# pdh930105/ARCQuant

Measured on AMD Instinct MI355X. Metric: ARC-NVFP4 GEMM TFLOP/s (M=4096, N=KQ=4096, KE=64), higher is better.
Workload: dtype f16

## Files before the change

arcquant_amd/agemm.py:

```python
from __future__ import annotations

import functools

import torch

from . import _lib
from ._lib import VARIANT_G16, VARIANT_G32, OUT_BF16, OUT_F32, ArcqError

_raw_stream = getattr(torch._C, "_cuda_getCurrentRawStream", None)


def _stream(t: torch.Tensor) -> int:
    if _raw_stream is not None:
        return _raw_stream(t.get_device())
    return torch.cuda.current_stream(t.device).cuda_stream


class _on:
    __slots__ = ("ctx",)

    def __init__(self, device):
        idx = device.index
        self.ctx = None if idx is None or idx == torch.cuda.current_device() else torch.cuda.device(device)

# ... 1 lines not shown
        if self.ctx is not None:
            self.ctx.__enter__()

    def __exit__(self, *exc):
        if self.ctx is not None:
            return self.ctx.__exit__(*exc)
        return False



def _need(t: torch.Tensor, dtype, name: str, ndim=None):
    if getattr(t, "dtype", None) is not dtype:
        raise RuntimeError(f"agemm: {name} must be a {dtype} tensor, got {getattr(t, 'dtype', type(t))}")
    if ndim is not None and t.dim() != ndim:
        raise RuntimeError(f"agemm: {name} must be {ndim}-D, got shape {tuple(t.shape)}")
    if not t.is_contiguous():
        raise RuntimeError(f"agemm: {name} must be contiguous")


def _opt(t, dtype, name, shape):
    if t is None:
        return None
    _need(t, dtype, name, len(shape))
    if t.shape != shape:
        raise RuntimeError(f"agemm: {name} must have shape {shape}")
    return t.data_ptr()


def _slots(t, who):
    if t is None:
        return None, 0
    _need(t, torch.int32, "absmax_slots", 1)
    if t.numel() == 0:
        raise RuntimeError(f"agemm.{who}: absmax_slots must not be empty")
    return t.data_ptr(), t.numel()


def _alpha(scale, scale_host):
    if isinstance(scale, torch.Tensor) and scale.is_cuda and scale.dtype == torch.float32 and scale.numel() == 1:
        return float(scale_host), scale, scale.data_ptr()
    return float(scale_host) * float(scale), None, None


def _alpha_as_f32(scale, scale_host):
    if isinstance(scale, torch.Tensor) and scale.is_cuda:
        scale = scale.reshape(-1)[:1].to(torch.float32)
        return float(scale_host), scale, scale.data_ptr()
    return float(scale_host) * float(scale), None, None


_OUT_CODES = {torch.bfloat16: OUT_BF16, torch.float32: OUT_F32}


def _out(out, M, N, out_dtype, like, who):
    code = _OUT_CODES.get(out_dtype)
    if code is None:
        raise RuntimeError(f"agemm.{who}: out_dtype must be bfloat16 or float32")
    if out is None:
        return torch.empty((M, N), dtype=out_dtype, device=like.device), code
    _need(out, out_dtype, "out", 2)
    if out.shape != (M, N):
        raise RuntimeError(f"agemm.{who}: out has the wrong shape, expected ({M}, {N})")
    return out, code


def _same_device(who: str, A: torch.Tensor, *ts):
    idx = A.get_device()
    if idx < 0:
        raise RuntimeError(f"agemm.{who}: the operands must live on the GPU (there is no CPU path)")
    for t in ts:
        if t is not None and t.get_device() != idx:
            raise RuntimeError(f"agemm.{who}: every operand must live on the GPU of the first one ({A.device}), got {t.device}")


def _debug_set_tile_overlap_tail(mode: int) -> None:
    fn = _lib.lib().arcq_debug_set_tile_overlap_tail
    fn.restype, fn.argtypes = None, [_lib._i32]
    fn(int(mode))
    rw_route.cache_clear()


def _debug_set_tile_pair_loads(on: int) -> None:
    fn = _lib.lib().arcq_debug_set_tile_pair_loads
    fn.restype, fn.argtypes = None, [_lib._i32]
    fn(int(on))


@functools.lru_cache(maxsize=None)
def variant_for_kq(KQ: int) -> int:
    return int(_lib.lib().arcq_variant_for_kq(int(KQ)))


@functools.lru_cache(maxsize=None)
def sf_buffer_bytes(rows: int, K: int) -> int:
    return int(_lib.lib().arcq_sf_alloc_bytes(int(rows), int(K)))


@functools.lru_cache(maxsize=None)
def _sf_used(rows: int, K: int) -> int:
    return int(_lib.lib().arcq_sf_used_bytes(int(rows), int(K)))


@functools.lru_cache(maxsize=None)
def _repacked_bytes(N: int, K: int):
    L = _lib.lib()
    return int(L.arcq_repacked_w_bytes(N, K)), int(L.arcq_repacked_sf_bytes(N, K))


def _need_repacked(RW, RSF, SFA, M, N, K, who, n_mult=1):
    _need(RW, torch.uint8, "RW", 1)
    _need(RSF, torch.uint8, "RSF", 1)
    if K % 64 or N % n_mult or (RW.numel(), RSF.numel()) != _repacked_bytes(N, K):
        raise RuntimeError(f"Value error in {who}: RW / RSF do not belong to a [{N}, {K}] weight" + (f", or N % {n_mult} != 0" if n_mult > 1 else ""))
    if SFA is not None and SFA.numel() < _sf_used(M, K):
        raise RuntimeError(f"Value error in {who}: SFA smaller than the swizzled layout of A")


def _quantize(fn_name: str, X: torch.Tensor, reorder_index: torch.Tensor, KE: int, variant):
    _need(X, torch.bfloat16, "X" if fn_name.endswith("_x") else "W", 2)
    _need(reorder_index, torch.int16, "reorder_index", 1)
    rows, KQ = X.shape
    KE = int(KE)
    if reorder_index.numel() != KQ:
        raise RuntimeError(f"agemm: reorder_index has {reorder_index.numel()} entries, expected {KQ}")
    K = KQ + KE
    if variant is None:
        variant = variant_for_kq(KQ)
    if KQ % 64 or KE % 64 or KE < 0 or KE > KQ:
        raise RuntimeError(f"Value error in {fn_name}: KQ={KQ}, KE={KE} is not valid")
    _same_device(fn_name, X, reorder_index)
    Q = torch.empty((rows, K // 2), dtype=torch.uint8, device=X.device)
    SF = torch.empty((sf_buffer_bytes(rows, K),), dtype=torch.uint8, device=X.device)
    L = _lib.lib()
    fn = L.arcq_quantize_x if fn_name.endswith("_x") else L.arcq_quantize_w
    with _on(X.device):
        st = fn(X.data_ptr(), reorder_index.data_ptr(), Q.data_ptr(), SF.data_ptr(), rows, KQ, KE, int(variant), _stream(X))
    _lib.check(st, fn_name)
    return Q, SF


def reorder_quantize_x(X: torch.Tensor, reorder_index: torch.Tensor, KE: int, variant=None):
    return _quantize("reorder_quantize_x", X, reorder_index, KE, variant)


def reorder_quantize_w(W: torch.Tensor, reorder_index: torch.Tensor, KE: int, variant=None):
    return _quantize("reorder_quantize_w", W, reorder_index, KE, variant)


def rmsnorm_quantize_x(X: torch.Tensor, W: torch.Tensor, eps: float, reorder_index: torch.Tensor, KE: int, variant=None):
    _need(X, torch.bfloat16, "X", 2)
    _need(W, torch.bfloat16, "W", 1)
    _need(reorder_index, torch.int16, "reorder_index", 1)
    M, KQ = X.shape
    KE = int(KE)
    K = KQ + KE
    if W.numel() != KQ or reorder_index.numel() != KQ:
        raise RuntimeError("agemm: rmsnorm weight / reorder_index length must equal X.shape[1]")
    if variant is None:
        variant = variant_for_kq(KQ)
    if KQ % 64 or KE % 64 or KE < 0 or KE > KQ or not (2048 <= KQ <= 8192):
        raise RuntimeError(f"Value error in run_rmsnorm_x_bf16_nvfp4: K value is not valid: {KQ}")
    _same_device("rmsnorm_quantize_x", X, W, reorder_index)
    QX = torch.empty((M, K // 2), dtype=torch.uint8, device=X.device)
    SFX = torch.empty((sf_buffer_bytes(M, K),), dtype=torch.uint8, device=X.device)
    with _on(X.device):
        st = _lib.lib().arcq_rmsnorm_quantize_x(X.data_ptr(), W.data_ptr(), float(eps), reorder_index.data_ptr(), QX.data_ptr(),
# ... 427 lines not shown
```

arcquant_amd/csrc/arcq_internal.hpp:

```cpp
#pragma once
#include <hip/hip_runtime.h>
#include <stdint.h>
#include <stdlib.h>

#include "../../include/arcq.h"

namespace arcq {

int fail(int code, const char* fmt, ...) __attribute__((format(printf, 2, 3)));

inline int env_int(const char* name, int dflt) {
  const char* e = getenv(name);
  return e ? atoi(e) : dflt;
}

constexpr int kMaxDevices = 64;
struct LdsOptIn {
  int granted[kMaxDevices];
};
int ensure_dynamic_lds(const void* kernel, LdsOptIn& cache, int bytes, const char* who);

struct LdsBytes {
  int launch, optin;
  LdsBytes(int bytes) : launch(bytes), optin(bytes) {}
// ... 42 lines not shown
int mx_quantize_w(const void* W, const int16_t* idx, uint8_t* QW, uint8_t* SFW, int64_t N, int64_t KQ, int64_t KE, hipStream_t stream);
int gemm_mx(const uint8_t* A, const uint8_t* B, const uint8_t* SFA, const uint8_t* SFB, void* D, int64_t M, int64_t N, int64_t Kp,
            float alpha_host, const float* alpha_dev, const void* bias, const void* residual, int out_dtype, hipStream_t stream);
int mx_rmsnorm_quantize_x(const void* X, const void* Wn, float eps, const int16_t* idx, uint8_t* QX, uint8_t* SFX, int64_t M, int64_t KQ,
                          int64_t KE, hipStream_t stream);
int mx_silu_mul_quantize_x(const void* GU, const int16_t* idx, uint8_t* QX, uint8_t* SFX, int64_t M, int64_t KQ, int64_t KE, int layout,
                           hipStream_t stream);
int gemm_mx_silu_mul(const uint8_t* A, const uint8_t* B, const uint8_t* SFA, const uint8_t* SFB, void* ACT, int64_t M, int64_t N, int64_t Kp,
                     float alpha_host, const float* alpha_dev, const void* bias, hipStream_t stream);
int gemm_mx_silu_mul_quantize(const uint8_t* A, const uint8_t* B, const uint8_t* SFA, const uint8_t* SFB, uint8_t* QACT, uint8_t* SFACT, int64_t M,
                              int64_t N, int64_t Kp, float alpha_host, const float* alpha_dev, const void* bias, int64_t KE, hipStream_t stream);

struct GemmArgs {
  const uint8_t* A;
  const uint8_t* B;
  const uint8_t* SFA;
  const uint8_t* SFB;
  void* D;
  int M, N, K;
  float alpha_host;
  const float* alpha_dev;
  const uint16_t* bias;
  const uint16_t* residual;
  int out_dtype;
  void* workspace;
  int64_t workspace_bytes;
  int epilogue = 0;
  unsigned int* absmax_slots = nullptr;
  int b_layout = 0;
};
template <typename Params>
void copy_gemm_fields(Params& p, const GemmArgs& a) {
  p.A = a.A; p.SFA = a.SFA; p.D = a.D;
  p.alpha_dev = a.alpha_dev; p.bias = a.bias; p.residual = a.residual;
  p.M = a.M; p.N = a.N; p.K = a.K; p.alpha_host = a.alpha_host; p.out_dtype = a.out_dtype;
}
enum : int { kEpiPlain = 0, kEpiSiluMul = 1 };
enum : int { kBRef = 0, kBRepacked = 1 };
int64_t gemm_silu_slots(int64_t M, int64_t N, int64_t K);
int64_t gemm_repacked_w_bytes(int64_t N, int64_t K);
int64_t gemm_repacked_sf_bytes(int64_t N, int64_t K);
int gemm_repacked_supported(int64_t M, int64_t N, int64_t K);
int gemm_repacked(const GemmArgs& a, const uint8_t* RW, const uint8_t* RSF, hipStream_t stream);
int gemm_repacked_mid_supported(int64_t M, int64_t N, int64_t K);
int gemm_repacked_mid(const GemmArgs& a, const uint8_t* RW, const uint8_t* RSF, hipStream_t stream);
int gemm_repacked_stream(const GemmArgs& a, const uint8_t* RW, const uint8_t* RSF, hipStream_t stream);
struct FusedArgs {
  int kind;
  int silu_act;
  const uint16_t* X;
  const uint16_t* Wn;
  float eps;
  const int16_t* idx;
  const uint32_t* in_slots;
  int n_in_slots;
  float* scale_out;
  const uint8_t* RW;
  const uint8_t* RSF;
  void* D;
  uint32_t* out_slots;
  const int16_t* act_scatter;
  int M, N, KQ, KE, variant;
  float alpha_host;
  const float* alpha_dev;
  const uint16_t* bias;
  const uint16_t* residual;
  int out_dtype;
};
int gemm_fused_supported(int kind, int64_t M, int64_t N, int64_t KQ, int64_t KE);
int gemm_fused(const FusedArgs& f, hipStream_t stream);
int64_t gemm_skinny_workspace_bytes(int64_t M, int64_t N, int64_t K);
int64_t gemm_tile_workspace_bytes(int64_t M, int64_t N, int64_t K);
int64_t gemm_tile_silu_slots(int64_t M, int64_t N, int64_t K);
int64_t gemm_decode_silu_slots(int64_t M, int64_t N, int64_t K);
int gemm_splitk_finish(const GemmArgs& a, int splitk, hipStream_t stream);
int gemm_skinny(const GemmArgs& a, hipStream_t stream);
int64_t gemm_decode_workspace_bytes(int64_t M, int64_t N, int64_t K);
int gemm_decode(const GemmArgs& a, hipStream_t stream);
int gemm_tile(const GemmArgs& a, hipStream_t stream);
int gemm_tile_repacked(const GemmArgs& a, hipStream_t stream);
int tile_overlap_tail_mode();
inline bool tile_overlap_tail_forced(int64_t M, int64_t N) { return tile_overlap_tail_mode() == 2 && M % 256 == 0 && N % 256 == 0; }
int tile_pair_loads_mode();
int gemm_regtile_cfg(int64_t M, int64_t N, int64_t K, int epilogue);
int gemm_regtile(const GemmArgs& a, int cfg, hipStream_t stream);
int gemm_regtile_fits(int64_t M, int64_t N, int64_t K, int b_layout);

struct KvWriteArgs {
  void* kv_data;
  void* kv_param;
  const int32_t *kv_indptr, *kv_indices, *last_page_offset;
  const void *k, *v, *k_param, *v_param;
  const int32_t* seqlen_indptr;
  int64_t ntok, B, L, layer, N, P;
  int format, dtype;
  bool quantize;
};
int kv_write(const KvWriteArgs& a, hipStream_t stream);
struct KvDecodeArgs {
  void* o;
  const void *q, *kv_data, *kv_param;
  const int32_t *kv_indptr, *kv_indices, *last_page_offset;
  int64_t B, Nq, L, layer, N, P, nnz;
  int format, dtype;
  void* workspace;
};
int kv_decode_splits(int64_t B, int64_t Nq, int64_t N, int64_t nnz, int64_t P);
int kv_decode(const KvDecodeArgs& a, hipStream_t stream);
struct KvStepArgs {
  const void *k, *v;
  int64_t q_stride, kv_stride;
  void* state;
};
int64_t kv_decode_chunks(int64_t Nq, int64_t N);
int kv_decode_step(const KvDecodeArgs& a, const KvStepArgs& st, hipStream_t stream);

struct KvPrefillArgs {
  void* o;
  const void* q;
  const int32_t* qo_indptr;
  const void *kv_data, *kv_param;
  const int32_t *kv_indptr, *kv_indices, *last_page_offset;
  int64_t ntok, B, Nq, L, layer, N, P;
  int dtype;
};
int kv_prefill(const KvPrefillArgs& a, hipStream_t stream);

struct KvRopeArgs {
  KvWriteArgs w;
  void* q_out;
  const void* q;
  const void *cos, *sin;
  int64_t q_stride, kv_stride, Nq;
  const char* who;
};
int kv_rope_write(const KvRopeArgs& a, hipStream_t stream);
struct RopeQkArgs {
  void *q, *k;
  const int32_t* positions;
  const void *cos, *sin;
  int64_t q_stride, k_stride, ntok, n_pos, Nq, N;
  int dtype;
};
int kv_rope_qk(const RopeQkArgs& a, hipStream_t stream);

}
```

arcquant_amd/csrc/gemm_tile_body.inc:

```
  constexpr int kThreads = WAVES_M * WAVES_N * 64;
  constexpr int WM = BM / WAVES_M, WN = BN / WAVES_N;
  constexpr int kT = kMfma32 ? 32 : 16;
  constexpr int TM = WM / kT, TN = WN / kT;
  using acc_t = typename std::conditional<kMfma32, f32x16, f32x4>::type;
  constexpr int A_UNITS = (BM * 2 + kThreads - 1) / kThreads, B_UNITS = (BN * 2 + kThreads - 1) / kThreads;
  constexpr bool A_PARTIAL = (BM * 2) % kThreads != 0, B_PARTIAL = (BN * 2) % kThreads != 0;
  static_assert(!A_PARTIAL || A_UNITS == 1, "a partial A pass is a single pass");
  static_assert(!B_PARTIAL || B_UNITS == 1, "a partial B pass is a single pass");
  constexpr int A_TILE = BM * kRowBytes, B_TILE = BN * kRowBytes;

  extern __shared__ __attribute__((aligned(16))) unsigned char smem[];
  unsigned char* const lds_a0 = smem;
  unsigned char* const lds_b0 = smem + A_TILE;
  unsigned char* const lds_a1 = smem + A_TILE + B_TILE;
  unsigned char* const lds_b1 = smem + 2 * A_TILE + B_TILE;

  const int ntiles = p.tiles_m * p.tiles_n;
  int bid = blockIdx.x, split = 0;
  if (p.splits > 1) {
    split = bid / ntiles;
    bid -= split * ntiles;
  }
  {
    const int q8 = ntiles >> 3, r8 = ntiles & 7, x = bid & 7, j = bid >> 3;
// ... 51 lines not shown
  int b_slot[B_UNITS][4];
#pragma unroll
  for (int u = 0; u < B_UNITS; ++u) {
    const int unit = tid + u * kThreads, r = B_PARTIAL ? min(unit >> 1, BN - 1) : unit >> 1, h = unit & 1;
    const int row = n0 + r, rc = row < p.N ? row : p.N - 1;
    if constexpr (kBLayout == kBRepacked) {
      const uint32_t rb = (uint32_t)((rc >> 4) - (n0 >> 4));
      b_q[u] = rb * (uint32_t)rw_tiles * 1024u + h * 256 + (rc & 15) * 16;
      b_sf[u] = rb * (uint32_t)rw_tiles * 128u + h * 64 + (rc & 15) * 4;
    } else {
      b_q[u] = (uint32_t)(rc - n0) * (uint32_t)half_k + h * 16;
      b_sf[u] = (uint32_t)(sf_atom_offset(rc, 0, atoms_k) - sf_atom_offset(n0, 0, atoms_k)) + h * 2;
    }
    b_live[u] = row < p.N ? kSfLive : 0u;
#pragma unroll
    for (int j = 0; j < 4; ++j) b_slot[u][j] = kMfma32 ? lds_slot32(r, h * 4 + j) : lds_slot(r, h * 4 + j);
  }
  const int fa_base = kMfma32 ? lds_slot32(wr * WM + (lane & 31), lane >> 5) : lds_slot(wr * WM + (lane & 15), lane >> 4);
  const int fb_base = kMfma32 ? lds_slot32(wc * WN + (lane & 31), lane >> 5) : lds_slot(wc * WN + (lane & 15), lane >> 4);
  acc_t acc[TM][TN];
  if constexpr (!kOverlapTail) {
#pragma unroll
    for (int i = 0; i < TM; ++i)
#pragma unroll
      for (int j = 0; j < TN; ++j)
#pragma unroll
        for (int r = 0; r < (kMfma32 ? 16 : 4); ++r) acc[i][j][r] = 0.f;
  }

  Staged sa[A_UNITS], sb[B_UNITS];
  auto load_step = [&](int atom) {
    atom = __builtin_amdgcn_readfirstlane(atom);
    const StageStep sa_step = stage_step(atom), sb_step = kBLayout == kBRepacked ? stage_step_rw(atom) : sa_step;
#pragma unroll
    for (int u = 0; u < A_UNITS; ++u) sa[u] = stage_load(a_src, a_q[u], a_sf[u], sa_step);
#pragma unroll
    for (int u = 0; u < B_UNITS; ++u) sb[u] = stage_load(b_src, b_q[u], b_sf[u], sb_step);
  };
#ifdef ARCQ_TILE_BODY_PAIR_LOADS
  Staged sa2[A_UNITS], sb2[B_UNITS];
  auto load_pair = [&](int atom0, int atom1, Staged (&a0)[A_UNITS], Staged (&b0)[B_UNITS], Staged (&a1)[A_UNITS], Staged (&b1)[B_UNITS], auto parts) {
    constexpr int kParts = decltype(parts)::value;
    atom0 = __builtin_amdgcn_readfirstlane(atom0);
    atom1 = __builtin_amdgcn_readfirstlane(atom1);
    const StageStep a_s0 = stage_step(atom0), a_s1 = stage_step(atom1);
    const StageStep b_s0 = kBLayout == kBRepacked ? stage_step_rw(atom0) : a_s0, b_s1 = kBLayout == kBRepacked ? stage_step_rw(atom1) : a_s1;
    __builtin_amdgcn_sched_barrier(0);
    if constexpr ((kParts & 1) != 0) {
#pragma unroll
      for (int u = 0; u < A_UNITS; ++u) {
        a0[u].q = stage_load_q(a_src, a_q[u], a_s0);
        __builtin_amdgcn_sched_barrier(0);
        a1[u].q = stage_load_q(a_src, a_q[u], a_s1);
        __builtin_amdgcn_sched_barrier(0);
      }
    }
    if constexpr ((kParts & 2) != 0) {
#pragma unroll
      for (int u = 0; u < B_UNITS; ++u) {
        b0[u].q = stage_load_q(b_src, b_q[u], b_s0);
        __builtin_amdgcn_sched_barrier(0);
        b1[u].q = stage_load_q(b_src, b_q[u], b_s1);
        __builtin_amdgcn_sched_barrier(0);
      }
    }
    if constexpr ((kParts & 4) != 0) {
#pragma unroll
      for (int u = 0; u < A_UNITS; ++u) {
        a0[u].sf = stage_load_sf(a_src, a_sf[u], a_s0);
        a1[u].sf = stage_load_sf(a_src, a_sf[u], a_s1);
      }
#pragma unroll
      for (int u = 0; u < B_UNITS; ++u) {
        b0[u].sf = stage_load_sf(b_src, b_sf[u], b_s0);
        b1[u].sf = stage_load_sf(b_src, b_sf[u], b_s1);
      }
    }
  };
  using kPairA = std::integral_constant<int, 1>;
  using kPairB = std::integral_constant<int, 2>;
  using kPairSf = std::integral_constant<int, 4>;
  using kPairAll = std::integral_constant<int, 7>;
#endif
  auto store_step = [&](unsigned char* la, unsigned char* lb) {
#pragma unroll
    for (int u = 0; u < A_UNITS; ++u)
      if (!A_PARTIAL || tid < BM * 2) stage_store(la, a_slot[u], sa[u], a_live[u]);
#pragma unroll
    for (int u = 0; u < B_UNITS; ++u)
      if (!B_PARTIAL || tid < BN * 2) stage_store(lb, b_slot[u], sb[u], b_live[u]);
  };
  auto mma_step = [&](const unsigned char* la, const unsigned char* lb) {
    if constexpr (kMfma32) {
#pragma unroll
      for (int ks = 0; ks < 4; ++ks) {
        Frag8 fa[TM], fb[TN];
#pragma unroll
        for (int i = 0; i < TM; ++i) fa[i].u = *reinterpret_cast<const uint4*>(la + (fa_base ^ (ks * 32)) + i * 32 * kRowBytes);
#pragma unroll
        for (int j = 0; j < TN; ++j) fb[j].u = *reinterpret_cast<const uint4*>(lb + (fb_base ^ (ks * 32)) + j * 32 * kRowBytes);
#pragma unroll
        for (int i = 0; i < TM; ++i)
#pragma unroll
          for (int j = 0; j < TN; ++j) acc[i][j] = __builtin_amdgcn_mfma_f32_32x32x16_f16(fb[j].v, fa[i].v, acc[i][j], 0, 0, 0);
      }
    } else {
#pragma unroll
      for (int ks = 0; ks < 2; ++ks) {
        Frag8 fa[TM], fb[TN];
#pragma unroll
        for (int i = 0; i < TM; ++i) fa[i].u = *reinterpret_cast<const uint4*>(la + (fa_base ^ (ks * 64)) + i * 16 * kRowBytes);
#pragma unroll
        for (int j = 0; j < TN; ++j) fb[j].u = *reinterpret_cast<const uint4*>(lb + (fb_base ^ (ks * 64)) + j * 16 * kRowBytes);
#pragma unroll
        for (int i = 0; i < TM; ++i)
#pragma unroll
          for (int j = 0; j < TN; ++j) acc[i][j] = __builtin_amdgcn_mfma_f32_16x16x32_f16(fb[j].v, fa[i].v, acc[i][j], 0, 0, 0);
      }
    }
  };
  const bool late = kStagger && wave >= 4;
  auto k_step = [&](int kt, unsigned char* ca, unsigned char* cb, unsigned char* na, unsigned char* nb) {
    Staged ta[A_UNITS], tb[B_UNITS];
#pragma unroll
    for (int u = 0; u < A_UNITS; ++u) ta[u] = sa[u];
#pragma unroll
    for (int u = 0; u < B_UNITS; ++u) tb[u] = sb[u];
    load_step(min(kt + 2 + (late ? 1 : 0), a_end - 1));
    __builtin_amdgcn_sched_barrier(0);
    mma_step(ca, cb);
    if (kStagger && late) __syncthreads();
    unsigned char* const wa = late ? ca : na;
    unsigned char* const wb = late ? cb : nb;
#pragma unroll
    for (int u = 0; u < A_UNITS; ++u)
      if (!A_PARTIAL || tid < BM * 2) stage_store(wa, a_slot[u], ta[u], a_live[u]);
#pragma unroll
    for (int u = 0; u < B_UNITS; ++u)
      if (!B_PARTIAL || tid < BN * 2) stage_store(wb, b_slot[u], tb[u], b_live[u]);
    if (!kStagger || !late) __syncthreads();
  };

  constexpr int kRot = 1;
  constexpr bool kRotate = kPipe && !kMfma32 && TM == 8 && TN == 4 && WAVES_M * WAVES_N == 8 && !A_PARTIAL && !B_PARTIAL;
  auto rd_frag = [&](const unsigned char* tile, int base, int ks, int i) { Frag8 f; f.u = *reinterpret_cast<const uint4*>(tile + (base ^ (ks * 64)) + i * 16 * kRowBytes); return f; };
  [[maybe_unused]] Frag8 head_b[TN], head_a[2];
  using kStepOne = std::integral_constant<int, 0>;
  using kStepPair = std::integral_constant<int, 1>;
  using kStepOdd = std::integral_constant<int, 2>;
  using kStepNone = std::integral_constant<int, 3>;
  auto k_step_pipe = [&](int kt, unsigned char* ca, unsigned char* cb, unsigned char* na, unsigned char* nb, auto step_kind) {
    static_assert(kMfma32 || TM % 2 == 0, "pairs of A fragments");
    constexpr int kKind = decltype(step_kind)::value;
    static_assert(kKind == 0 || kPairLoads, "the paired-load sibling's steps");
    Staged ta[A_UNITS], tb[B_UNITS];
#pragma unroll
    for (int u = 0; u < A_UNITS; ++u) ta[u] = sa[u];
#pragma unroll
    for (int u = 0; u < B_UNITS; ++u) tb[u] = sb[u];
    if constexpr (kKind == kStepOne::value) load_step(min(kt + 2, a_end - 1));
#ifdef ARCQ_TILE_BODY_PAIR_LOADS
    if constexpr (kKind == kStepOdd::value) {
#pragma unroll
      for (int u = 0; u < A_UNITS; ++u) ta[u] = sa2[u];
#pragma unroll
      for (int u = 0; u < B_UNITS; ++u) tb[u] = sb2[u];
    }
    if constexpr (kKind == kStepPair::value) load_pair(min(kt + 2, a_end - 1), min(kt + 3, a_end - 1), sa2, sb2, sa, sb, kPairA{});
#endif
    __builtin_amdgcn_sched_barrier(0);
    constexpr int kPieces = (A_UNITS + B_UNITS) * 4, kBlocks = kMfma32 ? 4 : TM;
    auto pieces = [&](int blk) {
#pragma unroll
      for (int c = blk; c < kPieces; c += kBlocks) {
        const int u = c >> 2, j = c & 3;
        if (u < A_UNITS) {
          if (!A_PARTIAL || tid < BM * 2) stage_piece(na, a_slot[u < A_UNITS ? u : 0][j], ta[u < A_UNITS ? u : 0], a_live[u < A_UNITS ? u : 0], j);
        } else {
          const int v = u - A_UNITS < B_UNITS ? u - A_UNITS : 0;
          if (!B_PARTIAL || tid < BN * 2) stage_piece(nb, b_slot[v][j], tb[v], b_live[v], j);
        }
      }
    };
    if constexpr (kMfma32) {
      Frag8 f32a[2][TM], f32b[2][TN];
      auto rd_set = [&](int buf, int ks) {
#pragma unroll
        for (int i = 0; i < TM; ++i) f32a[buf][i].u = *reinterpret_cast<const uint4*>(ca + (fa_base ^ (ks * 32)) + i * 32 * kRowBytes);
#pragma unroll
        for (int j = 0; j < TN; ++j) f32b[buf][j].u = *reinterpret_cast<const uint4*>(cb + (fb_base ^ (ks * 32)) + j * 32 * kRowBytes);
      };
      rd_set(0, 0);
#pragma unroll
      for (int ks = 0; ks < 4; ++ks) {
        if (ks + 1 < 4) rd_set((ks + 1) & 1, ks + 1);
        __builtin_amdgcn_sched_barrier(0);
#pragma unroll
        for (int i = 0; i < TM; ++i)
#pragma unroll
          for (int j = 0; j < TN; ++j)
            if constexpr (kMfma32)
              acc[i][j] = __builtin_amdgcn_mfma_f32_32x32x16_f16(f32b[ks & 1][j].v, f32a[ks & 1][i].v, acc[i][j], 0, 0, 0);
        pieces(ks);
        __builtin_amdgcn_sched_barrier(0);
      }
      __syncthreads();
      return;
    }
    auto rd_a = [&](int ks, int i) { return rd_frag(ca, fa_base, ks, i); };
    auto rd_b = [&](int ks, int j) { return rd_frag(cb, fb_base, ks, j); };
    if constexpr (kRotate) {
      constexpr int kQ = 2 * (TM / 2), kHalf = TM / 2, kLast = kQ - 1 - kRot, kNPre = kLast + 1;
      static_assert(kRot >= 1 && kLast >= kHalf, "the second K half's B fragments are read ahead of the barrier, a block before their use");
      auto read_by = [](int b) { const int extra = b - (kLast - kRot), h = b + 1 + (extra > 0 ? extra : 0); return h < kQ - 1 ? h : kQ - 1; };
      Frag8 fb1[TN], fq[kQ][2];
      fq[0][0] = head_a[0];
      fq[0][1] = head_a[1];
#pragma unroll
      for (int q = 0; q < kQ; ++q) {
        const int ks = q / kHalf, pr = q % kHalf;
        constexpr int kHeadReads = TN + 2;
        int n_pieces = 0, n_reads = 0;
#ifdef ARCQ_TILE_BODY_PAIR_LOADS
        if constexpr (kKind == kStepPair::value) {
          if (q == 2) load_pair(min(kt + 2, a_end - 1), min(kt + 3, a_end - 1), sa2, sb2, sa, sb, kPairB{});
          if (q == 4) load_pair(min(kt + 2, a_end - 1), min(kt + 3, a_end - 1), sa2, sb2, sa, sb, kPairSf{});
          if (q == 2 || q == 4) __builtin_amdgcn_sched_barrier(0);
        }
#endif
        if (q <= kLast) {
#pragma unroll
          for (int r = (q ? read_by(q - 1) : 0) + 1; r <= read_by(q); ++r) {
            fq[r][0] = rd_a(r / kHalf, 2 * (r % kHalf));
            fq[r][1] = rd_a(r / kHalf, 2 * (r % kHalf) + 1);
          }
          if (q == kHalf - 1) {
#pragma unroll
            for (int j = 0; j < TN; ++j) fb1[j] = rd_b(1, j);
          }
        }
        __builtin_amdgcn_sched_barrier(0);
#pragma unroll
        for (int ii = 0; ii < 2; ++ii)
#pragma unroll
          for (int j = 0; j < TN; ++j)
            acc[2 * pr + ii][j] = __builtin_amdgcn_mfma_f32_16x16x32_f16((ks ? fb1[j] : head_b[j]).v, fq[q][ii].v, acc[2 * pr + ii][j], 0, 0, 0);
        if (q <= kLast) {
#pragma unroll
          for (int c = 0; c < kPieces; ++c)
            if (c * kNPre / kPieces == q) {
              const int u = c >> 2, j = c & 3;
              if (u < A_UNITS) {
                if (j == 0) asm volatile("" : "+v"(ta[u].sf));
                stage_piece(na, a_slot[u][j], ta[u], a_live[u], j);
              } else {
                if (j == 0) asm volatile("" : "+v"(tb[u - A_UNITS].sf));
                stage_piece(nb, b_slot[u - A_UNITS][j], tb[u - A_UNITS], b_live[u - A_UNITS], j);
              }
              ++n_pieces;
            }
        } else {
          const int i0 = q - kLast - 1;
#pragma unroll
          for (int n = i0 * kHeadReads / kRot; n < (i0 + 1) * kHeadReads / kRot; ++n) {
            if (n < TN) head_b[n] = rd_frag(nb, fb_base, 0, n);
            else head_a[n - TN] = rd_frag(na, fa_base, 0, n - TN);
            ++n_reads;
          }
        }
#pragma unroll
        for (int m8 = 0; m8 < 2 * TN; ++m8) {
          __builtin_amdgcn_sched_group_barrier(0x008, 1, 0);
          if (q <= kLast) {
            if (n_pieces == 1) __builtin_amdgcn_sched_group_barrier(0x002, 2, 0);
            else if (n_pieces == 2) __builtin_amdgcn_sched_group_barrier(0x002, 4, 0);
            else if (n_pieces >= 3) __builtin_amdgcn_sched_group_barrier(0x002, 6, 0);
          } else if (m8 < n_reads) {
            __builtin_amdgcn_sched_group_barrier(0x100, 1, 0);
          }
        }
        __builtin_amdgcn_sched_barrier(0);
        if (q == kLast) {
          __syncthreads();
          __builtin_amdgcn_sched_barrier(0);
        }
      }
      return;
    }
    constexpr int kPairs = TM / 2, kSeq = 2 * kPairs, kAhead = 1;
    Frag8 fb[2][TN], fq[kSeq][2];
    auto rd_pair = [&](int q) {
      fq[q][0] = rd_a(q / kPairs, 2 * (q % kPairs));
      fq[q][1] = rd_a(q / kPairs, 2 * (q % kPairs) + 1);
    };
#pragma unroll
    for (int j = 0; j < TN; ++j) fb[0][j] = rd_b(0, j);
#pragma unroll
    for (int q = 0; q < kAhead; ++q) rd_pair(q);
#pragma unroll
    for (int q = 0; q < kSeq; ++q) {
      const int ks = q / kPairs, pr = q % kPairs;
      if (q + kAhead < kSeq) rd_pair(q + kAhead);
      if (ks == 0 && pr == kPairs - 1 - (kAhead - 1 < kPairs - 1 ? kAhead - 1 : kPairs - 1)) {
#pragma unroll
        for (int j = 0; j < TN; ++j) fb[1][j] = rd_b(1, j);
      }
      __builtin_amdgcn_sched_barrier(0);
#pragma unroll
      for (int ii = 0; ii < 2; ++ii)
#pragma unroll
        for (int j = 0; j < TN; ++j)
          if constexpr (!kMfma32)
            acc[2 * pr + ii][j] = __builtin_amdgcn_mfma_f32_16x16x32_f16(fb[ks][j].v, fq[q][ii].v, acc[2 * pr + ii][j], 0, 0, 0);
      pieces(q);
#pragma unroll
      for (int m8 = 0; m8 < (TM == 8 ? 2 * TN : 0); ++m8) {
        __builtin_amdgcn_sched_group_barrier(0x008, 1, 0);
        __builtin_amdgcn_sched_group_barrier(0x002, 2, 0);
      }
      __builtin_amdgcn_sched_barrier(0);
    }
    __syncthreads();
  };

#ifdef ARCQ_TILE_BODY_PAIR_LOADS
  Staged sa0[A_UNITS], sb0[B_UNITS];
  load_pair(a_begin, min(a_begin + 1, a_end - 1), sa0, sb0, sa, sb, kPairAll{});
#else
  load_step(a_begin);
  Staged sa0[A_UNITS], sb0[B_UNITS];
#pragma unroll
  for (int u = 0; u < A_UNITS; ++u) sa0[u] = sa[u];
#pragma unroll
  for (int u = 0; u < B_UNITS; ++u) sb0[u] = sb[u];
  load_step(min(a_begin + 1, a_end - 1));
#endif
  __builtin_amdgcn_sched_barrier(0);
  if constexpr (kOverlapTail) {
#pragma unroll
    for (int i = 0; i < TM; ++i)
#pragma unroll
      for (int j = 0; j < TN; ++j) {
        acc[i][j] = acc_t{};
        asm volatile("" : "+v"(acc[i][j]));
      }
    __builtin_amdgcn_sched_barrier(0);
  }
#pragma unroll
  for (int u = 0; u < A_UNITS; ++u)
    if (!A_PARTIAL || tid < BM * 2) stage_store(lds_a0, a_slot[u], sa0[u], a_live[u]);
#pragma unroll
  for (int u = 0; u < B_UNITS; ++u)
    if (!B_PARTIAL || tid < BN * 2) stage_store(lds_b0, b_slot[u], sb0[u], b_live[u]);
  if (kStagger && late) {
    store_step(lds_a1, lds_b1);
    load_step(min(a_begin + 2, a_end - 1));
  }
  __syncthreads();
  if constexpr (kRotate) {
#pragma unroll
    for (int j = 0; j < TN; ++j) head_b[j] = rd_frag(lds_b0, fb_base, 0, j);
    head_a[0] = rd_frag(lds_a0, fa_base, 0, 0);
    head_a[1] = rd_frag(lds_a0, fa_base, 0, 1);
  }
  int kt = a_begin;
  float alpha_dev = 1.0f;
  if (p.alpha_dev) alpha_dev = *reinterpret_cast<const __attribute__((address_space(4))) float*>(reinterpret_cast<uintptr_t>(p.alpha_dev));
  asm volatile("" : "+s"(alpha_dev));
  if (WAVES_M * WAVES_N == 8 && wave >= 4) __builtin_amdgcn_s_setprio(1);
  ARCQ_TILE_STAMP(1);
  [[maybe_unused]] int tail_buf = 0;
  if constexpr (kOverlapTail) {
    static_assert(kRotate, "the final step is entered with head fragments");
    using Even = std::conditional_t<kPairLoads, kStepPair, kStepOne>;
    using Odd = std::conditional_t<kPairLoads, kStepOdd, kStepOne>;
    using Last = std::conditional_t<kPairLoads, kStepNone, kStepOne>;
    for (; kt + 2 < a_end; kt += 2) {
      k_step_pipe(kt, lds_a0, lds_b0, lds_a1, lds_b1, Even{});
      k_step_pipe(kt + 1, lds_a1, lds_b1, lds_a0, lds_b0, Odd{});
    }
    if (kt + 1 < a_end) {
      k_step_pipe(kt, lds_a0, lds_b0, lds_a1, lds_b1, Last{});
      tail_buf = A_TILE + B_TILE;
    }
  } else if constexpr (kPipe) {
    for (; kt + 1 < a_end; kt += 2) {
      k_step_pipe(kt, lds_a0, lds_b0, lds_a1, lds_b1, kStepOne{});
      k_step_pipe(kt + 1, lds_a1, lds_b1, lds_a0, lds_b0, kStepOne{});
    }
    if (kt < a_end) k_step_pipe(kt, lds_a0, lds_b0, lds_a1, lds_b1, kStepOne{});
  } else {
    for (; kt + 1 < a_end; kt += 2) {
      k_step(kt, lds_a0, lds_b0, lds_a1, lds_b1);
      k_step(kt + 1, lds_a1, lds_b1, lds_a0, lds_b0);
    }
    if (kt < a_end) k_step(kt, lds_a0, lds_b0, lds_a1, lds_b1);
  }
  if constexpr (!kOverlapTail) ARCQ_TILE_STAMP(2);

  const float alpha = p.alpha_host * alpha_dev;
  const bool vec_ok = (p.N & 3) == 0;
  uint32_t act_max = 0;
  [[maybe_unused]] auto interior_epilogue = [&](auto has_bias, auto has_res) __attribute__((always_inline)) {
    constexpr bool kBias = decltype(has_bias)::value, kRes = decltype(has_res)::value;
    constexpr bool kSilu = kEpi == kEpiSiluMul;
    constexpr uint32_t kElem = kSilu ? 1 : 2;
    unsigned char* const tile_d = reinterpret_cast<unsigned char*>(p.D) + ((size_t)m0 * p.N + n0) * kElem;
    const unsigned char* const tile_r = kRes ? reinterpret_cast<const unsigned char*>(p.residual) + ((size_t)m0 * p.N + n0) * 2 : nullptr;
    uint32_t t = tid;
    asm volatile("" : "+v"(t));
    const uint32_t lane_row = (t >> 6) / WAVES_N * WM + (t & 15), lane_col = (t >> 6) % WAVES_N * WN + 4 * ((t >> 4) & 3);
    uint32_t off = lane_row * (uint32_t)p.N + lane_col;
    const uint32_t row_step = 16u * (uint32_t)p.N;
    constexpr bool kWide = !kSilu && TN % 2 == 0;
    typedef uint32_t u32x4_a8 __attribute__((ext_vector_type(4), aligned(8)));
    [[maybe_unused]] const uint32_t g4 = (t >> 4) & 3;
    [[maybe_unused]] uint32_t off_w = off - 4 * g4 + ((g4 & 1) ? 16 + 4 * (g4 - 1) : 4 * g4);
    [[maybe_unused]] uint2 held = make_uint2(0, 0);
    constexpr bool kPackedBias = kOverlapTail && kBias && kRes;
    float bias_f[TN][4];
    [[maybe_unused]] uint2 bias_v[TN];
    if constexpr (kBias) {
#pragma unroll
      for (int j = 0; j < TN; ++j) {
        const uint2 b = *reinterpret_cast<const uint2*>(p.bias + n0 + lane_col + j * 16);
        if constexpr (kPackedBias) {
          bias_v[j] = b;
        } else {
          bias_f[j][0] = bf16_bits_to_f32(b.x & 0xffffu); bias_f[j][1] = bf16_bits_to_f32(b.x >> 16);
          bias_f[j][2] = bf16_bits_to_f32(b.y & 0xffffu); bias_f[j][3] = bf16_bits_to_f32(b.y >> 16);
        }
      }
    }
    uint2 res_cur[TN], res_nxt[TN];
    auto res_load = [&](uint32_t o, uint2 (&r)[TN]) {
#pragma unroll
      for (int j = 0; j < TN; ++j) r[j] = *reinterpret_cast<const uint2*>(tile_r + (size_t)o * 2 + j * 32);
    };
    if constexpr (kRes) res_load(off, res_cur);
    auto row_quad = [&](int i, int j) __attribute__((always_inline)) {
      {
        if constexpr (kPackedBias) {
          uint2 b = bias_v[j];
          asm volatile("" : "+v"(b.x), "+v"(b.y));
          bias_f[j][0] = bf16_bits_to_f32(b.x & 0xffffu); bias_f[j][1] = bf16_bits_to_f32(b.x >> 16);
          bias_f[j][2] = bf16_bits_to_f32(b.y & 0xffffu); bias_f[j][3] = bf16_bits_to_f32(b.y >> 16);
        }
        float d[4] = {alpha * acc[i][j][0], alpha * acc[i][j][1], alpha * acc[i][j][2], alpha * acc[i][j][3]};
        if constexpr (kSilu) {
          if constexpr (kBias) {
#pragma unroll
            for (int r = 0; r < 4; r += 2) {
              round2_to_bf16(d[r], d[r + 1]);
              d[r] += bias_f[j][r];
              d[r + 1] += bias_f[j][r + 1];
            }
          }
          const uint32_t y01 = pack_bf16x2_hw(d[0], d[1]), y23 = pack_bf16x2_hw(d[2], d[3]);
          const uint32_t a0 = silu_mul_bf16(y01 & 0xffffu, y01 >> 16), a1 = silu_mul_bf16(y23 & 0xffffu, y23 >> 16);
          *reinterpret_cast<uint32_t*>(tile_d + (size_t)off + j * 16) = a0 | (a1 << 16);
          act_max = max(act_max, max(a0 & 0x7fffu, a1 & 0x7fffu));
        } else {
          if constexpr (kBias) {
#pragma unroll
            for (int r = 0; r < 4; r += 2) {
              round2_to_bf16(d[r], d[r + 1]);
// ... 233 lines not shown
```

arcquant_amd/csrc/gemm_tile_common.hpp:

```cpp
#pragma once
#include <hip/hip_runtime.h>
#include <stdint.h>

#include "arcq_internal.hpp"
#include "gemm_common.hpp"

namespace arcq {

struct TileParams {
  const uint8_t* A;
  const uint8_t* B;
  const uint8_t* SFA;
  const uint8_t* SFB;
  void* D;
  const float* alpha_dev;
  const uint16_t* bias;
  const uint16_t* residual;
  int M, N, K;
  float alpha_host;
  int out_dtype;
  int tiles_m, tiles_n;
  int splits, atoms_per_split;
  float* partial;
  int epi;
  unsigned int* slots;
#ifdef ARCQ_STREAM_STAMPS
  unsigned long long* stamps;
#endif
};
constexpr int kTileStamps = 5;
int launch_tile_overlap_tail(const TileParams& p, int epi, int b_layout, dim3 grid, hipStream_t stream);
int launch_tile_pair_loads(const TileParams& p, int b_layout, dim3 grid, hipStream_t stream);

#pragma GCC visibility push(hidden)
struct TileCfg { int id, bm, bn, waves; };
const TileCfg& tile_cfg(int id);
bool tile_stagger();
bool tile_pipe();
void tile_split(int64_t M, int64_t N, int64_t K, int BM, int BN, int* splits, int* atoms_per_split);
int effective_cfg(int64_t M, int64_t N, int64_t K, bool* may_split);
#ifdef ARCQ_STREAM_STAMPS
extern unsigned long long* g_tile_stamps;
#endif
#pragma GCC visibility pop

#ifdef ARCQ_STREAM_STAMPS
#define ARCQ_TILE_STAMP(k)                                                                                     \
  do {                                                                                                         \
    if (p.stamps && tid == 0) {                                                                                \
      unsigned long long t0_, t1_;                                                                             \
      asm volatile("s_memtime %0\n\ts_memrealtime %1\n\ts_waitcnt lgkmcnt(0)" : "=s"(t0_), "=s"(t1_)::"memory"); \
      p.stamps[(size_t)blockIdx.x * (2 * kTileStamps) + 2 * (k)] = t0_;                                        \
      p.stamps[(size_t)blockIdx.x * (2 * kTileStamps) + 2 * (k) + 1] = t1_;                                    \
    }                                                                                                          \
  } while (0)
#else
#define ARCQ_TILE_STAMP(k) do { } while (0)
#endif

constexpr int kBK = 64;
constexpr int kRowBytes = kBK * 2;

__device__ __forceinline__ int lds_slot(int r, int ks) { return r * kRowBytes + ((ks ^ (r & 7)) << 4); }
__device__ __forceinline__ int lds_slot32(int r, int ks) { return r * kRowBytes + ((ks ^ ((r >> 1) & 7)) << 4); }

struct Staged {
  uint4 q;
  uint32_t sf;
};

typedef uint32_t u32x4 __attribute__((ext_vector_type(4)));
typedef __amdgpu_buffer_rsrc_t buf_rsrc;

__device__ __forceinline__ buf_rsrc stage_rsrc(const uint8_t* base, uint32_t bytes) {
  return __builtin_amdgcn_make_buffer_rsrc(const_cast<uint8_t*>(base), 0, (int)bytes, 0x00020000);
}

struct StageSrc {
  buf_rsrc q, sf;
};
struct StageStep {
  uint32_t q, sf;
};
__device__ __forceinline__ StageStep stage_step(int atom) { return {(uint32_t)atom * 32u, (uint32_t)atom * 512u}; }
__device__ __forceinline__ StageStep stage_step_rw(int atom) {
  return {(uint32_t)atom * 512u, (uint32_t)((atom >> 2) * 256 + (atom & 1) * 128 + ((atom >> 1) & 1) * 2)};
}
__device__ __forceinline__ Staged stage_load(const StageSrc& src, uint32_t q_lane, uint32_t sf_lane, StageStep step) {
  Staged s;
  const u32x4 q = __builtin_amdgcn_raw_buffer_load_b128(src.q, (int)q_lane, (int)step.q, 0);
  s.q = make_uint4(q.x, q.y, q.z, q.w);
  s.sf = (uint16_t)__builtin_amdgcn_raw_buffer_load_b16(src.sf, (int)sf_lane, (int)step.sf, 0);
  return s;
}
__device__ __forceinline__ uint4 stage_load_q(const StageSrc& src, uint32_t q_lane, StageStep step) {
  const u32x4 q = __builtin_amdgcn_raw_buffer_load_b128(src.q, (int)q_lane, (int)step.q, 0);
  return make_uint4(q.x, q.y, q.z, q.w);
}
__device__ __forceinline__ uint32_t stage_load_sf(const StageSrc& src, uint32_t sf_lane, StageStep step) {
  return (uint16_t)__builtin_amdgcn_raw_buffer_load_b16(src.sf, (int)sf_lane, (int)step.sf, 0);
}

constexpr uint32_t kSfLive = 0x3f803f80u;
__device__ __forceinline__ f16x2 sf_pair_both(uint32_t sf16, uint32_t live_mask) {
  const uint32_t w = ((sf16 << 7) | (sf16 << 15)) & live_mask;
  f16x2 r;
  __builtin_memcpy(&r, &w, 4);
  return r;
}
template <int kHalf>
__device__ __forceinline__ f16x2 sf_splat(f16x2 s) { return __builtin_shufflevector(s, s, kHalf, kHalf); }

__device__ __forceinline__ void stage_piece(unsigned char* tile, int slot, const Staged& s, uint32_t live_mask, int j) {
  const uint32_t w = j == 0 ? s.q.x : j == 1 ? s.q.y : j == 2 ? s.q.z : s.q.w;
  const f16x2 sf = sf_pair_both(s.sf, live_mask);
// ... 17 lines not shown
```

arcquant_amd/csrc/gemm_tile_launch.hpp:

```cpp
#pragma once
#include <hip/hip_runtime.h>
#include <stdint.h>

#include <type_traits>

#include "arcq_internal.hpp"
#include "gemm_common.hpp"
#include "gemm_tile_common.hpp"

namespace arcq {

template <int BM, int BN, int WAVES_M, int WAVES_N, bool kMfma32, int kEpi, bool kStagger, bool kPipe, int kBLayout = kBRef>
__global__ __launch_bounds__(WAVES_M* WAVES_N * 64) void gemm_tile_kernel(TileParams p) {
  constexpr bool kOverlapTail = false, kPairLoads = false;
  [[maybe_unused]] constexpr int kEpiOps = 0;
#include "gemm_tile_body.inc"
}

template <int BM, int BN, int WAVES_M, int WAVES_N, bool kMfma32 = false, int kEpi = kEpiPlain, int kBLayout = kBRef>
static int launch_tile(const GemmArgs& a, hipStream_t stream, bool allow_split = false) {
  TileParams p;
  copy_gemm_fields(p, a);
  p.B = a.B; p.SFB = a.SFB;
  p.tiles_m = (a.M + BM - 1) / BM;
  p.tiles_n = (a.N + BN - 1) / BN;
  p.splits = 1; p.atoms_per_split = a.K / 64; p.partial = nullptr;
  p.epi = a.epilogue; p.slots = a.absmax_slots;
#ifdef ARCQ_STREAM_STAMPS
  p.stamps = g_tile_stamps;
#endif
  if (allow_split && a.epilogue == kEpiPlain) {
    tile_split(a.M, a.N, a.K, BM, BN, &p.splits, &p.atoms_per_split);
    if (p.splits > 1) {
      const int64_t need = (int64_t)p.splits * a.M * a.N * (int64_t)sizeof(float);
      if (!a.workspace || a.workspace_bytes < need)
        return fail(ARCQ_ERR_WORKSPACE, "arcq_gemm_nvfp4: split-K needs %lld B of workspace, got %lld", (long long)need,
                    (long long)a.workspace_bytes);
      p.partial = reinterpret_cast<float*>(a.workspace);
    }
  }
  if (((int64_t)a.K + 255) / 256 * 256 * 128 > 0xffffffffll)
    return fail(ARCQ_ERR_SHAPE, "arcq_gemm_nvfp4 (tile): K = %lld: a tile's rows of an operand exceed 32-bit offsets", (long long)a.K);
  const int lds = 2 * (BM + BN) * kRowBytes;
  const dim3 grid((unsigned)(p.tiles_m * p.tiles_n * p.splits)), block(WAVES_M * WAVES_N * 64);
  const char* who = "arcq_gemm_nvfp4 (tile)";
  constexpr bool kCanStagger = WAVES_M * WAVES_N == 8 && BM == 256 && BN == 256;
  const bool pipe = tile_pipe(), stagger = !pipe && kCanStagger && tile_stagger();
  int rc;
  bool overlap_tail = false;
  if constexpr (BM == 256 && BN == 256 && WAVES_M * WAVES_N == 8 && !kMfma32)
    overlap_tail = pipe && (kEpi == kEpiSiluMul ? tile_overlap_tail_mode() == 2 : tile_overlap_tail_mode() != 0) && a.M % BM == 0 && a.N % BN == 0 && p.splits <= 1 && a.out_dtype == ARCQ_OUT_BF16 &&
                   (int64_t)BM * a.N < (1ll << 31) && ((reinterpret_cast<uintptr_t>(a.bias) | reinterpret_cast<uintptr_t>(a.residual)) & 7) == 0;
  if (overlap_tail && kEpi == kEpiPlain && tile_pair_loads_mode() != 0) rc = launch_tile_pair_loads(p, kBLayout, grid, stream);
  else if (overlap_tail) rc = launch_tile_overlap_tail(p, kEpi, kBLayout, grid, stream);
  else if (!pipe && !stagger) rc = launch_kernel<gemm_tile_kernel<BM, BN, WAVES_M, WAVES_N, kMfma32, kEpi, false, false, kBLayout>>(grid, block, lds, stream, who, p);
  else if (pipe) rc = launch_kernel<gemm_tile_kernel<BM, BN, WAVES_M, WAVES_N, kMfma32, kEpi, false, true, kBLayout>>(grid, block, lds, stream, who, p);
  else rc = launch_kernel<gemm_tile_kernel<BM, BN, WAVES_M, WAVES_N, kMfma32, kEpi, kCanStagger, false, kBLayout>>(grid, block, lds, stream, who, p);
  if (rc != ARCQ_OK) return rc;
  if (p.splits > 1) return gemm_splitk_finish(a, p.splits, stream);
  return ARCQ_OK;
}

template <int kEpi, int kBLayout>
static int gemm_tile_epi(const GemmArgs& a, hipStream_t stream) {
  bool sp;
  switch (effective_cfg(a.M, a.N, a.K, &sp)) {
    case 1: case 9: return launch_tile<128, 128, 2, 2, false, kEpi, kBLayout>(a, stream, sp);
    case 2: return launch_tile<256, 256, 2, 2, false, kEpi, kBLayout>(a, stream);
    case 4: return launch_tile<128, 256, 2, 2, false, kEpi, kBLayout>(a, stream);
    case 5: return launch_tile<256, 256, 2, 4, true, kEpi, kBLayout>(a, stream);
    case 6: return launch_tile<128, 128, 2, 2, true, kEpi, kBLayout>(a, stream);
    case 7: return launch_tile<64, 256, 1, 4, false, kEpi, kBLayout>(a, stream, sp);
    case 8: return launch_tile<32, 256, 1, 4, false, kEpi, kBLayout>(a, stream, sp);
    case 10: return launch_tile<128, 256, 2, 4, false, kEpi, kBLayout>(a, stream, sp);
    case 11: return launch_tile<256, 128, 4, 2, false, kEpi, kBLayout>(a, stream, sp);
    case 12: return launch_tile<128, 128, 2, 4, false, kEpi, kBLayout>(a, stream, sp);
    case 13: return launch_tile<64, 256, 1, 8, false, kEpi, kBLayout>(a, stream, sp);
    case 14: return launch_tile<64, 128, 2, 4, false, kEpi, kBLayout>(a, stream, sp);
    case 15: return launch_tile<64, 64, 2, 2, false, kEpi, kBLayout>(a, stream, sp);
    case 16: return launch_tile<64, 128, 2, 2, false, kEpi, kBLayout>(a, stream, sp);
    case 17: return launch_tile<128, 64, 2, 2, false, kEpi, kBLayout>(a, stream, sp);
    default: return launch_tile<256, 256, 2, 4, false, kEpi, kBLayout>(a, stream);
  }
}

}
```

Baseline: 1530.

## Add quad-step global load prefetch kernel for 256x256 tile GEMM

Result: faster. 1551, median of 6 (+1.4%).

```diff
diff --git a/arcquant_amd/agemm.py b/arcquant_amd/agemm.py
--- a/arcquant_amd/agemm.py
+++ b/arcquant_amd/agemm.py
@@ -107,6 +107,12 @@
 
 def _debug_set_tile_pair_loads(on: int) -> None:
     fn = _lib.lib().arcq_debug_set_tile_pair_loads
+    fn.restype, fn.argtypes = None, [_lib._i32]
+    fn(int(on))
+
+
+def _debug_set_tile_quad_loads(on: int) -> None:
+    fn = _lib.lib().arcq_debug_set_tile_quad_loads
     fn.restype, fn.argtypes = None, [_lib._i32]
     fn(int(on))
 
diff --git a/arcquant_amd/csrc/arcq_internal.hpp b/arcquant_amd/csrc/arcq_internal.hpp
--- a/arcquant_amd/csrc/arcq_internal.hpp
+++ b/arcquant_amd/csrc/arcq_internal.hpp
@@ -148,6 +148,7 @@
 int tile_overlap_tail_mode();
 inline bool tile_overlap_tail_forced(int64_t M, int64_t N) { return tile_overlap_tail_mode() == 2 && M % 256 == 0 && N % 256 == 0; }
 int tile_pair_loads_mode();
+int tile_quad_loads_mode();
 int gemm_regtile_cfg(int64_t M, int64_t N, int64_t K, int epilogue);
 int gemm_regtile(const GemmArgs& a, int cfg, hipStream_t stream);
 int gemm_regtile_fits(int64_t M, int64_t N, int64_t K, int b_layout);
diff --git a/arcquant_amd/csrc/gemm_tile_body.inc b/arcquant_amd/csrc/gemm_tile_body.inc
--- a/arcquant_amd/csrc/gemm_tile_body.inc
+++ b/arcquant_amd/csrc/gemm_tile_body.inc
@@ -157,6 +157,36 @@
   using kPairSf = std::integral_constant<int, 4>;
   using kPairAll = std::integral_constant<int, 7>;
 #endif
+#ifdef ARCQ_TILE_BODY_QUAD_LOADS
+  static_assert(kBLayout == kBRef, "quads follow the reference layout's rows (repacked launches keep gemm_tile_pl_kernel)");
+  Staged qa[4][A_UNITS], qb[4][B_UNITS];
+  Staged yb[2][B_UNITS];
+  bool quad_single = false;
+  auto quad_steps = [&](int atom0, StageStep (&s)[4]) {
+#pragma unroll
+    for (int i = 0; i < 4; ++i) s[i] = stage_step(__builtin_amdgcn_readfirstlane(min(atom0 + i, a_end - 1)));
+  };
+  auto load_quad_q = [&](int atom0, const StageSrc& src, const auto& lane_q, auto& dst) {
+    StageStep s[4];
+    quad_steps(atom0, s);
+    __builtin_amdgcn_sched_barrier(0);
+#pragma unroll
+    for (int u = 0; u < (int)(sizeof(dst[0]) / sizeof(dst[0][0])); ++u)
+#pragma unroll
+      for (int i = 0; i < 4; ++i) {
+        dst[i][u].q = stage_load_q(src, lane_q[u], s[i]);
+        __builtin_amdgcn_sched_barrier(0);
+      }
+  };
+  auto load_quad_sf = [&](int atom0, const StageSrc& src, const auto& lane_sf, auto& dst, int first, int last) {
+    StageStep s[4];
+    quad_steps(atom0, s);
+#pragma unroll
+    for (int u = 0; u < (int)(sizeof(dst[0]) / sizeof(dst[0][0])); ++u)
+#pragma unroll
+      for (int i = first; i <= last; ++i) dst[i][u].sf = stage_load_sf(src, lane_sf[u], s[i]);
+  };
+#endif
   auto store_step = [&](unsigned char* la, unsigned char* lb) {
 #pragma unroll
     for (int u = 0; u < A_UNITS; ++u)
@@ -224,6 +254,13 @@
   using kStepPair = std::integral_constant<int, 1>;
   using kStepOdd = std::integral_constant<int, 2>;
   using kStepNone = std::integral_constant<int, 3>;
+#ifdef ARCQ_TILE_BODY_QUAD_LOADS
+  using kStepQuadA = std::integral_constant<int, 4>;
+  using kStepQuadB = std::integral_constant<int, 5>;
+  using kStepOneA = std::integral_constant<int, 6>;
+  using kStepSfA = std::integral_constant<int, 7>;
+  using kStepSfB = std::integral_constant<int, 8>;
+#endif
   auto k_step_pipe = [&](int kt, unsigned char* ca, unsigned char* cb, unsigned char* na, unsigned char* nb, auto step_kind) {
     static_assert(kMfma32 || TM % 2 == 0, "pairs of A fragments");
     constexpr int kKind = decltype(step_kind)::value;
@@ -242,6 +279,18 @@
       for (int u = 0; u < B_UNITS; ++u) tb[u] = sb2[u];
     }
     if constexpr (kKind == kStepPair::value) load_pair(min(kt + 2, a_end - 1), min(kt + 3, a_end - 1), sa2, sb2, sa, sb, kPairA{});
+#endif
+#ifdef ARCQ_TILE_BODY_QUAD_LOADS
+    if constexpr (kKind == kStepQuadA::value) load_quad_q(kt + 2, a_src, a_q, qa);
+    if constexpr (kKind == kStepSfA::value) load_quad_sf(kt + 1, a_src, a_sf, qa, 1, 3);
+    if constexpr (kKind == kStepSfB::value) load_quad_sf(kt + 1, b_src, b_sf, qb, 1, 3);
+    if constexpr (kKind == kStepOneA::value) {
+      if (quad_single) {
+        const StageStep one = stage_step(__builtin_amdgcn_readfirstlane(kt + 2));
+#pragma unroll
+        for (int u = 0; u < A_UNITS; ++u) qa[0][u] = stage_load(a_src, a_q[u], a_sf[u], one);
+      }
+    }
 #endif
     __builtin_amdgcn_sched_barrier(0);
     constexpr int kPieces = (A_UNITS + B_UNITS) * 4, kBlocks = kMfma32 ? 4 : TM;
@@ -300,6 +349,19 @@
         if constexpr (kKind == kStepPair::value) {
           if (q == 2) load_pair(min(kt + 2, a_end - 1), min(kt + 3, a_end - 1), sa2, sb2, sa, sb, kPairB{});
           if (q == 4) load_pair(min(kt + 2, a_end - 1), min(kt + 3, a_end - 1), sa2, sb2, sa, sb, kPairSf{});
+          if (q == 2 || q == 4) __builtin_amdgcn_sched_barrier(0);
+        }
+#endif
+#ifdef ARCQ_TILE_BODY_QUAD_LOADS
+        if constexpr (kKind == kStepQuadA::value) {
+          if (q == 2) {
+            load_quad_sf(kt + 2, a_src, a_sf, qa, 0, 0);
+            __builtin_amdgcn_sched_barrier(0);
+          }
+        }
+        if constexpr (kKind == kStepQuadB::value) {
+          if (q == 2) load_quad_q(kt + 2, b_src, b_q, qb);
+          if (q == 4) load_quad_sf(kt + 2, b_src, b_sf, qb, 0, 0);
           if (q == 2 || q == 4) __builtin_amdgcn_sched_barrier(0);
         }
 #endif
@@ -401,6 +463,17 @@
 #ifdef ARCQ_TILE_BODY_PAIR_LOADS
   Staged sa0[A_UNITS], sb0[B_UNITS];
   load_pair(a_begin, min(a_begin + 1, a_end - 1), sa0, sb0, sa, sb, kPairAll{});
+#ifdef ARCQ_TILE_BODY_QUAD_LOADS
+  {
+    const StageStep b_s2 = stage_step(__builtin_amdgcn_readfirstlane(min(a_begin + 2, a_end - 1)));
+    const StageStep b_s3 = stage_step(__builtin_amdgcn_readfirstlane(min(a_begin + 3, a_end - 1)));
+#pragma unroll
+    for (int u = 0; u < B_UNITS; ++u) {
+      yb[0][u] = stage_load(b_src, b_q[u], b_sf[u], b_s2);
+      yb[1][u] = stage_load(b_src, b_q[u], b_sf[u], b_s3);
+    }
+  }
+#endif
 #else
   load_step(a_begin);
   Staged sa0[A_UNITS], sb0[B_UNITS];
@@ -450,13 +523,55 @@
     using Even = std::conditional_t<kPairLoads, kStepPair, kStepOne>;
     using Odd = std::conditional_t<kPairLoads, kStepOdd, kStepOne>;
     using Last = std::conditional_t<kPairLoads, kStepNone, kStepOne>;
-    for (; kt + 2 < a_end; kt += 2) {
-      k_step_pipe(kt, lds_a0, lds_b0, lds_a1, lds_b1, Even{});
-      k_step_pipe(kt + 1, lds_a1, lds_b1, lds_a0, lds_b0, Odd{});
-    }
-    if (kt + 1 < a_end) {
-      k_step_pipe(kt, lds_a0, lds_b0, lds_a1, lds_b1, Last{});
-      tail_buf = A_TILE + B_TILE;
+#ifdef ARCQ_TILE_BODY_QUAD_LOADS
+    if constexpr (kQuadLoads) {
+      auto stage_from = [&](const Staged (&a)[A_UNITS], const Staged (&b)[B_UNITS]) {
+#pragma unroll
+        for (int u = 0; u < A_UNITS; ++u) sa[u] = a[u];
+#pragma unroll
+        for (int u = 0; u < B_UNITS; ++u) sb[u] = b[u];
+      };
+      for (; kt + 4 < a_end; kt += 4) {
+        k_step_pipe(kt, lds_a0, lds_b0, lds_a1, lds_b1, kStepQuadA{});
+        stage_from(qa[0], yb[0]);
+        k_step_pipe(kt + 1, lds_a1, lds_b1, lds_a0, lds_b0, kStepSfA{});
+        stage_from(qa[1], yb[1]);
+        k_step_pipe(kt + 2, lds_a0, lds_b0, lds_a1, lds_b1, kStepQuadB{});
+        stage_from(qa[2], qb[0]);
+        k_step_pipe(kt + 3, lds_a1, lds_b1, lds_a0, lds_b0, kStepSfB{});
+        stage_from(qa[3], qb[1]);
+#pragma unroll
+        for (int u = 0; u < B_UNITS; ++u) {
+          yb[0][u] = qb[2][u];
+          yb[1][u] = qb[3][u];
+        }
+      }
+      const int left = a_end - 1 - kt;
+      if (left >= 1) {
+        quad_single = left >= 2;
+        k_step_pipe(kt, lds_a0, lds_b0, lds_a1, lds_b1, kStepOneA{});
+        if (left >= 2) {
+          stage_from(qa[0], yb[0]);
+          quad_single = left >= 3;
+          k_step_pipe(kt + 1, lds_a1, lds_b1, lds_a0, lds_b0, kStepOneA{});
+          if (left >= 3) {
+            stage_from(qa[0], yb[1]);
+            k_step_pipe(kt + 2, lds_a0, lds_b0, lds_a1, lds_b1, kStepNone{});
+          }
+        }
+        if (left & 1) tail_buf = A_TILE + B_TILE;
+      }
+    } else
+#endif
+    {
+      for (; kt + 2 < a_end; kt += 2) {
+        k_step_pipe(kt, lds_a0, lds_b0, lds_a1, lds_b1, Even{});
+        k_step_pipe(kt + 1, lds_a1, lds_b1, lds_a0, lds_b0, Odd{});
+      }
+      if (kt + 1 < a_end) {
+        k_step_pipe(kt, lds_a0, lds_b0, lds_a1, lds_b1, Last{});
+        tail_buf = A_TILE + B_TILE;
+      }
     }
   } else if constexpr (kPipe) {
     for (; kt + 1 < a_end; kt += 2) {
diff --git a/arcquant_amd/csrc/gemm_tile_common.hpp b/arcquant_amd/csrc/gemm_tile_common.hpp
--- a/arcquant_amd/csrc/gemm_tile_common.hpp
+++ b/arcquant_amd/csrc/gemm_tile_common.hpp
@@ -31,6 +31,7 @@
 constexpr int kTileStamps = 5;
 int launch_tile_overlap_tail(const TileParams& p, int epi, int b_layout, dim3 grid, hipStream_t stream);
 int launch_tile_pair_loads(const TileParams& p, int b_layout, dim3 grid, hipStream_t stream);
+int launch_tile_quad_loads(const TileParams& p, dim3 grid, hipStream_t stream);
 
 #pragma GCC visibility push(hidden)
 struct TileCfg { int id, bm, bn, waves; };
diff --git a/arcquant_amd/csrc/gemm_tile_launch.hpp b/arcquant_amd/csrc/gemm_tile_launch.hpp
--- a/arcquant_amd/csrc/gemm_tile_launch.hpp
+++ b/arcquant_amd/csrc/gemm_tile_launch.hpp
@@ -51,7 +51,8 @@
   if constexpr (BM == 256 && BN == 256 && WAVES_M * WAVES_N == 8 && !kMfma32)
     overlap_tail = pipe && (kEpi == kEpiSiluMul ? tile_overlap_tail_mode() == 2 : tile_overlap_tail_mode() != 0) && a.M % BM == 0 && a.N % BN == 0 && p.splits <= 1 && a.out_dtype == ARCQ_OUT_BF16 &&
                    (int64_t)BM * a.N < (1ll << 31) && ((reinterpret_cast<uintptr_t>(a.bias) | reinterpret_cast<uintptr_t>(a.residual)) & 7) == 0;
-  if (overlap_tail && kEpi == kEpiPlain && tile_pair_loads_mode() != 0) rc = launch_tile_pair_loads(p, kBLayout, grid, stream);
+  if (overlap_tail && kEpi == kEpiPlain && kBLayout == kBRef && tile_pair_loads_mode() != 0 && tile_quad_loads_mode() != 0) rc = launch_tile_quad_loads(p, grid, stream);
+  else if (overlap_tail && kEpi == kEpiPlain && tile_pair_loads_mode() != 0) rc = launch_tile_pair_loads(p, kBLayout, grid, stream);
   else if (overlap_tail) rc = launch_tile_overlap_tail(p, kEpi, kBLayout, grid, stream);
   else if (!pipe && !stagger) rc = launch_kernel<gemm_tile_kernel<BM, BN, WAVES_M, WAVES_N, kMfma32, kEpi, false, false, kBLayout>>(grid, block, lds, stream, who, p);
   else if (pipe) rc = launch_kernel<gemm_tile_kernel<BM, BN, WAVES_M, WAVES_N, kMfma32, kEpi, false, true, kBLayout>>(grid, block, lds, stream, who, p);
diff --git a/arcquant_amd/csrc/gemm_tile_ql.hip b/arcquant_amd/csrc/gemm_tile_ql.hip
--- /dev/null
+++ b/arcquant_amd/csrc/gemm_tile_ql.hip
@@ -0,0 +1,36 @@
+#include <type_traits>
+
+#include "gemm_tile_common.hpp"
+
+namespace arcq {
+
+template <int BM, int BN, int WAVES_M, int WAVES_N, int kEpi, int kBLayout, int kEpiOps>
+__global__ __launch_bounds__(WAVES_M* WAVES_N * 64) void gemm_tile_ql_kernel(TileParams p) {
+  static_assert(kEpi == kEpiPlain && kBLayout == kBRef && kEpiOps >= 0 && kEpiOps < 4, "bit 0 bias, bit 1 residual; the reference layout's rows");
+  constexpr bool kMfma32 = false, kStagger = false, kPipe = true, kOverlapTail = true, kPairLoads = true, kQuadLoads = true;
+#define ARCQ_TILE_BODY_PAIR_LOADS
+#define ARCQ_TILE_BODY_QUAD_LOADS
+#include "gemm_tile_body.inc"
+#undef ARCQ_TILE_BODY_QUAD_LOADS
+#undef ARCQ_TILE_BODY_PAIR_LOADS
+}
+
+static int g_tile_quad_loads = 1;
+int tile_quad_loads_mode() { return g_tile_quad_loads; }
+extern "C" void arcq_debug_set_tile_quad_loads(int on) { g_tile_quad_loads = on != 0; }
+
+template <int kEpiOps>
+static int launch_ql(const TileParams& p, dim3 grid, hipStream_t stream) {
+  return launch_kernel<gemm_tile_ql_kernel<256, 256, 2, 4, kEpiPlain, kBRef, kEpiOps>>(grid, dim3(512), 2 * (256 + 256) * kRowBytes, stream,
+                                                                                     "arcq_gemm_nvfp4 (tile, quad loads)", p);
+}
+int launch_tile_quad_loads(const TileParams& p, dim3 grid, hipStream_t stream) {
+  switch ((p.bias ? 1 : 0) | (p.residual ? 2 : 0)) {
+    case 1: return launch_ql<1>(p, grid, stream);
+    case 2: return launch_ql<2>(p, grid, stream);
+    case 3: return launch_ql<3>(p, grid, stream);
+    default: return launch_ql<0>(p, grid, stream);
+  }
+}
+
+}
```
